# yyamamoto79/guetzli-cuda-opencl

Hardware: AMD Instinct MI355X
Metric: Mpixels/s end-to-end encode @ q=95; achieved HBM GB/s on Butteraugli pass (higher is better)
Workload: dtype f32

## Files before the change

guetzli-cuda-opencl_amd/csrc/kernels/butteraugli_kernels.inc:

```
#pragma once

namespace gz {




constexpr int kIdctM[64] = {
    8192, 11363, 10703, 9633,   8192,  6437,   4433,   2260,   8192, 9633,  4433,  -2259, -8192,
    -11362, -10704, -6436, 8192, 6437, -4433,  -11362, -8192, 2261,   10704,  9633, 8192,  2260,
    -10703, -6436, 8192, 9633,  -4433, -11363, 8192,   -2260, -10703, 6436,   8192, -9633, -4433,
    11363,  8192,  -6437, -4433, 11362, -8192, -2261,  10704, -9633,  8192,   -9633, 4433, 2259,
    -8192,  11362, -10704, 6436, 8192,  -11363, 10703, -9633, 8192,   -6437,  4433,  -2260,
};
typedef short c2l_v2s __attribute__((ext_vector_type(2)));
__device__ __forceinline__ int c2l_dot8(int r, const c2l_v2s (&v)[4], int bias) {
  int acc = bias;
#pragma unroll
  for (int k = 0; k < 4; ++k)
    acc = __builtin_amdgcn_sdot2(c2l_v2s{static_cast<short>(kIdctM[8 * r + 2 * k]),
                                         static_cast<short>(kIdctM[8 * r + 2 * k + 1])},
                                 v[k], acc, false);
  return acc;
}
constexpr int kC2lBlocks = 8;
// ... 166 lines not shown
  scales[static_cast<size_t>(blockIdx.y) * stride + pos] = blur_scale(c_tab.blur[sig], pos, size, &lo, &hi);
}

constexpr int kBlurTile = 256;
constexpr int kBlurLds = 1152;

struct RowsPlain {
  const float* in[kMaxBlurPlanes];
  int w;
  __device__ float at(int p, int y, int x) const { return in[p][static_cast<size_t>(y) * w + x]; }
  __device__ const float* row(int p, int y) const { return in[p] + static_cast<size_t>(y) * w; }
  __device__ static float get(const float* r, int x) { return r[x]; }
  static constexpr bool kPlain = true;
};
struct RowsDiffmap {
  const float* resval;
  int rw;
  __device__ float at(int, int y, int x) const { return resval[static_cast<size_t>(y / 3) * rw + x / 3]; }
  __device__ const float* row(int, int y) const { return resval + static_cast<size_t>(y / 3) * rw; }
  __device__ static float get(const float* r, int x) { return r[x / 3]; }
  static constexpr bool kPlain = false;
};

enum BlurStage : int {
  kBlurRefOpsin = 0, kBlurOpsin, kBlurEdge, kBlurLowFreq, kBlurMask, kBlurDiffmap,
  kBlurLfMask,
};

template <int kSig>
__host__ __device__ constexpr int blur_hstride(int dx) {
  return BlurGeom<kSig>::STEP > 1 ? (dx + 1) & ~1 : dx;
}

template <int kSig> struct HRowRep { static constexpr int N = 1; };
template <> struct HRowRep<kSigDiffmap> { static constexpr int N = 3; };

template <int kSig, int K>
struct H4Geom {
  static constexpr int STEP = BlurGeom<kSig>::STEP, R = BlurGeom<kSig>::R, NT = 2 * R + 1;
  static constexpr int OUT = 64 * K;
  static constexpr int SPAN = OUT * STEP + 2 * R;
  static constexpr int NV = (K + (NT - 1) / STEP + K - 1) / K;
  static constexpr int PMIN = OUT + K * NV;
  static constexpr int PST = STEP == 1 ? (PMIN + 3) / 4 * 4 : ((PMIN + 23) / 32) * 32 + 8;
  static constexpr int LDS = STEP * PST;
};
constexpr int kH4MaxLds = 688;
template <int kSig> struct H4K { static constexpr int K = 2; };

template <int kSig, int K, class Rows>
__device__ __forceinline__ void blur_h4_row(const Rows& rows, float* __restrict__ out, int p, int band,
                                            int y, int w, int lane,
                                            const float* __restrict__ scales, int stride,
                                            float* lds) {
  using G = H4Geom<kSig, K>;
  constexpr int STEP = G::STEP, R = G::R, NT = G::NT, NV = G::NV, PST = G::PST;
  constexpr int IT = (G::SPAN + 63) / 64;
  static_assert(G::LDS <= kH4MaxLds, "H4 LDS region");
  static_assert(K == 2 || K == 4, "2 or 4 outputs per lane");
  const BlurSpec& s = c_tab.blur[kSig];
  const int dx = (w + STEP - 1) / STEP;
  const int ox0 = band * G::OUT;
  const int x_begin = ox0 * STEP - R;
  const float* src = rows.row(p, kSig == kSigDiffmap ? 3 * y : y);
  float v[IT];
  if (Rows::kPlain && x_begin >= 0 && x_begin + IT * 64 <= w) {
    const float* b = src + x_begin + lane;
#pragma unroll
    for (int k = 0; k < IT; ++k) v[k] = b[64 * k];
  } else {
#pragma unroll
    for (int k = 0; k < IT; ++k) {
      const int e = lane + 64 * k, x = x_begin + e;
      const int xc = x < 0 ? 0 : (x < w ? x : w - 1);
      const float t = Rows::get(src, xc);
      v[k] = (e < G::SPAN && x >= 0 && x < w) ? t : 0.0f;
    }
  }
#pragma unroll
  for (int k = 0; k < IT; ++k) {
    const int e = lane + 64 * k;
    if (e < G::SPAN) lds[(e % STEP) * PST + e / STEP] = v[k];
  }
  __builtin_amdgcn_fence(__ATOMIC_RELEASE, "wavefront");
  __builtin_amdgcn_wave_barrier();
  __builtin_amdgcn_fence(__ATOMIC_ACQUIRE, "wavefront");
  float a[STEP][NV * K];
#pragma unroll
  for (int ph = 0; ph < STEP; ++ph)
#pragma unroll
    for (int m = 0; m < NV; ++m) {
      if constexpr (K == 4) {
        const float4 q = *reinterpret_cast<const float4*>(lds + ph * PST + 4 * lane + 4 * m);
        a[ph][4 * m] = q.x;
        a[ph][4 * m + 1] = q.y;
        a[ph][4 * m + 2] = q.z;
        a[ph][4 * m + 3] = q.w;
      } else {
        const float2 q = *reinterpret_cast<const float2*>(lds + ph * PST + 2 * lane + 2 * m);
        a[ph][2 * m] = q.x;
        a[ph][2 * m + 1] = q.y;
      }
    }
  f32x2 s01 = {0.0f, 0.0f}, s23 = {0.0f, 0.0f};
#pragma unroll
  for (int t = 0; t < NT; ++t) {
    const int ph = t % STEP, i = t / STEP;
    const float tap = s.taps[t];
    s01 += f32x2{a[ph][i], a[ph][i + 1]} * tap;
    if constexpr (K == 4) s23 += f32x2{a[ph][i + 2], a[ph][i + 3]} * tap;
  }
  const int ox = ox0 + K * lane;
  const float* sx = scales + static_cast<size_t>(kSig * 2) * stride + ox * STEP;
  float* o = out + static_cast<size_t>(y) * blur_hstride<kSig>(dx) + ox;
  const float r[4] = {s01.x, s01.y, s23.x, s23.y};
#pragma unroll
  for (int j = 0; j < K; ++j)
    if (ox + j < dx) o[j] = r[j] * sx[j * STEP];
}

template <int kStage, class Rows>
__global__ __launch_bounds__(256) void k_blur_h4(Rows rows, BlurPlanes bp, int w, int h,
                                                 const float* __restrict__ scales, int stride) {
  __shared__ __attribute__((aligned(16))) float lds[4][kH4MaxLds];
  const int wv = wave_id(), lane = threadIdx.x & 63;
  const int item = static_cast<int>(blockIdx.x) * 4 + wv;
  if (item >= bp.start[bp.nplanes]) return;
  int q = 0;
  while (q + 1 < bp.nplanes && item >= bp.start[q + 1]) ++q;
  const int local = item - bp.start[q];
  const int band = local % bp.tiles[q], y = local / bp.tiles[q];
#define GZ_H4(S) blur_h4_row<S, H4K<S>::K>(rows, bp.out[q], q, band, y, w, lane, scales, stride, lds[wv])
  if constexpr (kStage == kBlurLowFreq) {
    GZ_H4(kSigLowFreq);
  } else if constexpr (kStage == kBlurMask || kStage == kBlurLfMask) {
    switch (bp.sig[q]) {
      case kSigLowFreq: if constexpr (kStage == kBlurLfMask) GZ_H4(kSigLowFreq); break;
      case kSigMaskX: GZ_H4(kSigMaskX); break;
      case kSigMaskY: GZ_H4(kSigMaskY); break;
      case kSigMaskBSub: GZ_H4(kSigMaskBSub); break;
      default: GZ_H4(kSigMaskB); break;
    }
  } else {
    GZ_H4(kSigDiffmap);
  }
#undef GZ_H4
}

template <int kSig> struct VsRows { static constexpr int N = 8; };
template <> struct VsRows<kSigLowFreq> { static constexpr int N = 16; };
template <int kSig> struct VsAhead { static constexpr int N = 4; };
template <> struct VsAhead<kSigMaskX> { static constexpr int N = 2; };
constexpr int kVsCols = 128;
template <int kSig>
struct VsGeom {
  static constexpr int STEP = BlurGeom<kSig>::STEP, R = BlurGeom<kSig>::R;
  static constexpr int A = 2 * R / STEP + 1;
  static constexpr int S = VsRows<kSig>::N;
  static constexpr int PERIODS = S + A - 1;
};
template <int kSig>
__host__ __device__ constexpr int vstream_segments(int h) {
  return ((h + BlurGeom<kSig>::STEP - 1) / BlurGeom<kSig>::STEP + VsRows<kSig>::N - 1) /
         VsRows<kSig>::N;
}

template <int kSig>
__device__ __forceinline__ void vstream_load(const float* plane, int ds, int h, int y, int ox0,
                                             int ox1, f32x2* v) {
  const int yc = y < 0 ? 0 : (y < h ? y : h - 1);
  const float* r = row_ptr(plane, HRowRep<kSig>::N == 1 ? yc : yc / HRowRep<kSig>::N, ds);
  if constexpr (BlurGeom<kSig>::STEP > 1) {
    *v = *reinterpret_cast<const f32x2*>(r + static_cast<unsigned>(ox0));
  } else {
    *v = f32x2{r[static_cast<unsigned>(ox0)], r[static_cast<unsigned>(ox1)]};
  }
}

template <int kSig, bool kLut = false>
__device__ __forceinline__ void blur_vstream_item(const BlurPlanes& bp, int p, int local, int w,
                                                  int h, int lane, const float* __restrict__ scales,
                                                  int stride) {
  using G = VsGeom<kSig>;
  constexpr int STEP = G::STEP, R = G::R, A = G::A, S = G::S, kVsAhead = VsAhead<kSig>::N;
  const BlurSpec& s = c_tab.blur[kSig];
  const int dx = (w + STEP - 1) / STEP, dy = (h + STEP - 1) / STEP;
  const int segs = vstream_segments<kSig>(h);
  const int seg = local % segs, g = local / segs;
  const int ox = g * kVsCols + 2 * lane;
  const bool in0 = ox < dx, in1 = ox + 1 < dx;
  const int ds = blur_hstride<kSig>(dx);
  const int ox0 = in0 ? ox : (dx - 1) & ~(STEP > 1 ? 1 : 0), ox1 = in1 ? ox + 1 : dx - 1;
  const int oy0 = seg * S;
  const int y_first = oy0 * STEP - R;
  const float* plane = bp.in[p];
  const float* sy = scales + static_cast<size_t>(kSig * 2 + 1) * stride;
  float* out = bp.out[p] + ox;
  float* out2 = kLut && bp.out2[p] ? bp.out2[p] + ox : nullptr;
  const bool lut = kLut && out2 != nullptr;
  f32x2 acc[A];
#pragma unroll
  for (int k = 0; k < A; ++k) acc[k] = f32x2{0.0f, 0.0f};
  f32x2 q[kVsAhead][STEP];
#pragma unroll
  for (int k = 0; k < kVsAhead; ++k)
#pragma unroll
    for (int j = 0; j < STEP; ++j)
      vstream_load<kSig>(plane, ds, h, y_first + k * STEP + j, ox0, ox1, &q[k][j]);
  auto period = [&](int m, f32x2* qm) {
    f32x2 cur[STEP];
#pragma unroll
    for (int j = 0; j < STEP; ++j) {
      const int y = y_first + m * STEP + j;
      const bool yin = y >= 0 && y < h;
      cur[j] = f32x2{masked(qm[j].x, yin), masked(qm[j].y, yin)};
      vstream_load<kSig>(plane, ds, h, y + kVsAhead * STEP, ox0, ox1, &qm[j]);
    }
    acc[0] = f32x2{0.0f, 0.0f};
#pragma unroll
    for (int j = 0; j < STEP; ++j) {
#pragma unroll
      for (int d = 0; d < A; ++d) {
        const int t = d * STEP + j;
        if (t <= 2 * R) acc[d] += cur[j] * s.taps[t];
      }
    }
    const int o = m - (A - 1);
    if (o >= 0 && oy0 + o < dy && o < S) {
      const float sc = sy[(oy0 + o) * STEP];
      const size_t off = static_cast<size_t>(oy0 + o) * dx;
      float* po = out + off;
      const float v0 = acc[A - 1].x * sc, v1 = acc[A - 1].y * sc;
      if (lut) {
        const int c = kSig == kSigMaskX ? 0 : (kSig == kSigMaskY ? 1 : 2);
        float* pd = out2 + off;
        if (in0) mask_lut_pair(c, v0, &po[0], &pd[0]);
        if (in1) mask_lut_pair(c, v1, &po[1], &pd[1]);
      } else {
        if (in0) po[0] = v0;
        if (in1) po[1] = v1;
      }
    }
#pragma unroll
    for (int d = A - 1; d > 0; --d) acc[d] = acc[d - 1];
  };
  for (int m = 0; m < G::PERIODS; m += kVsAhead) {
#pragma unroll
    for (int k = 0; k < kVsAhead; ++k) period(m + k, q[k]);
  }
}

template <int kStage>
__global__ __launch_bounds__(256, 4) void k_blur_vstream(BlurPlanes bp, int w, int h,
                                                      const float* __restrict__ scales, int stride) {
  const int item = static_cast<int>(blockIdx.x) * 4 + wave_id();
  const int lane = threadIdx.x & 63;
  if (item >= bp.start[bp.nplanes]) return;
  int q = 0;
  while (q + 1 < bp.nplanes && item >= bp.start[q + 1]) ++q;
  const int local = item - bp.start[q];
#define GZ_VS(S) blur_vstream_item<S>(bp, q, local, w, h, lane, scales, stride)
#define GZ_VSL(S) blur_vstream_item<S, kStage == kBlurLfMask>(bp, q, local, w, h, lane, scales, stride)
  if constexpr (kStage == kBlurLowFreq) {
    GZ_VS(kSigLowFreq);
  } else if constexpr (kStage == kBlurMask || kStage == kBlurLfMask) {
    switch (bp.sig[q]) {
      case kSigLowFreq: if constexpr (kStage == kBlurLfMask) GZ_VS(kSigLowFreq); break;
      case kSigMaskX: GZ_VSL(kSigMaskX); break;
      case kSigMaskY: GZ_VSL(kSigMaskY); break;
      case kSigMaskBSub: GZ_VSL(kSigMaskBSub); break;
      default: GZ_VSL(kSigMaskB); break;
    }
  } else {
    GZ_VS(kSigDiffmap);
  }
#undef GZ_VS
#undef GZ_VSL
}

constexpr int kB2MaxR = 3;

struct Blur2DPlanes {
  const float* in[6];
  float* out[6];
  int sig[6];
  int nplanes, tiles_x, tiles_y;
};

constexpr int kBsCols = 64 - 2 * kB2MaxR, kBsPf = 8, kBsRows = 32;

template <int kSig>
__device__ __forceinline__ void blur_stream_strip(const float* __restrict__ in, float* __restrict__ out,
                                                  int w, int h, int x0, int y0, int rows, int lane,
                                                  const float* __restrict__ scales, int stride) {
  constexpr int R = BlurGeom<kSig>::R, NT = 2 * R + 1;
  const BlurSpec& s = c_tab.blur[kSig];
  const int x = x0 - kB2MaxR + lane;
  const bool xin = x >= 0 && x < w;
  const int xc = xin ? x : 0;
  const bool emit = lane >= kB2MaxR && lane < kB2MaxR + kBsCols && x < w;
  const float sxv = x < w ? scales[static_cast<size_t>(kSig * 2) * stride + xc] : 0.0f;
  const float* sy = scales + static_cast<size_t>(kSig * 2 + 1) * stride;
  const int y_end = min(y0 + rows, h);
  const int ya = y0 - R, yb = y_end + R;
  auto load = [&](int y) {
    const bool ok = xin && y >= 0 && y < h;
    const int yc = y < 0 ? 0 : (y < h ? y : h - 1);
    const float v = row_ptr(in, yc, w)[static_cast<unsigned>(xc)];
    return masked(v, ok);
  };
  float pm[kBsPf];
#pragma unroll
  for (int k = 0; k < kBsPf; ++k) pm[k] = load(ya + k);
  float hv[NT + 1];
#pragma unroll
  for (int t = 0; t <= NT; ++t) hv[t] = 0.0f;
  for (int y = ya; y < yb; y += 2) {
    const float m0 = pm[0], m1 = pm[1];
#pragma unroll
    for (int k = 0; k + 2 < kBsPf; ++k) pm[k] = pm[k + 2];
    pm[kBsPf - 2] = load(y + kBsPf);
    pm[kBsPf - 1] = load(y + kBsPf + 1);
    float a0[NT], a1[NT];
    a0[R] = m0;
    a1[R] = m1;
#pragma unroll
    for (int k = 1; k <= R; ++k) {
      a0[R + k] = wave_next(a0[R + k - 1]);
      a1[R + k] = wave_next(a1[R + k - 1]);
      a0[R - k] = wave_prev(a0[R - k + 1]);
      a1[R - k] = wave_prev(a1[R - k + 1]);
    }
    f32x2 hs = {0.0f, 0.0f};
#pragma unroll
    for (int t = 0; t < NT; ++t) hs += f32x2{a0[t], a1[t]} * s.taps[t];
    hs *= sxv;
#pragma unroll
    for (int t = 0; t + 2 <= NT; ++t) hv[t] = hv[t + 2];
    hv[NT - 1] = hs.x;
    hv[NT] = hs.y;
    const int yo = y - R;
    if (yo + 1 >= y0) {
      f32x2 acc = {0.0f, 0.0f};
#pragma unroll
      for (int t = 0; t < NT; ++t) acc += f32x2{hv[t], hv[t + 1]} * s.taps[t];
      if (emit && yo >= y0) row_ptr(out, yo, w)[static_cast<unsigned>(x)] = acc.x * sy[yo];
      if (emit && yo + 1 < y_end) row_ptr(out, yo + 1, w)[static_cast<unsigned>(x)] = acc.y * sy[yo + 1];
    }
  }
}

template <int kStage>
__global__ __launch_bounds__(256) void k_blur_stream(Blur2DPlanes bp, int w, int h, int rows,
                                                     const float* __restrict__ scales, int stride) {
  const int lane = threadIdx.x & 63, wv = wave_id();
  const int item = blockIdx.x * 4 + wv;
  const int per_plane = bp.tiles_x * bp.tiles_y;
  if (item >= bp.nplanes * per_plane) return;
  const int p = item / per_plane, t = item % per_plane;
  const int x0 = (t % bp.tiles_x) * kBsCols, y0 = (t / bp.tiles_x) * rows;
#define GZ_BS(S) blur_stream_strip<S>(bp.in[p], bp.out[p], w, h, x0, y0, rows, lane, scales, stride)
  switch (bp.sig[p]) {
    case kSigEdgeX: GZ_BS(kSigEdgeX); break;
    case kSigEdgeY: GZ_BS(kSigEdgeY); break;
    case kSigEdgeB: GZ_BS(kSigEdgeB); break;
    default: GZ_BS(kSigOpsin); break;
  }
#undef GZ_BS
}

constexpr int kOpTX = 64, kOpTY = 32, kOpR = 2;
constexpr int kOpInW = kOpTX + 2 * kOpR, kOpInH = kOpTY + 2 * kOpR;

__global__ __launch_bounds__(256) void k_opsin2d(const float* __restrict__ lin, int w, int h,
                                                 int tiles_x, float* __restrict__ xyb,
                                                 const float* __restrict__ scales, int stride) {
  __shared__ float in_t[kOpInH * kOpInW];
  __shared__ float h_t[3][kOpInH * kOpTX];
  const int x0 = (blockIdx.x % tiles_x) * kOpTX, y0 = (blockIdx.x / tiles_x) * kOpTY;
  const BlurSpec& s = c_tab.blur[kSigOpsin];
  const int ntap = 2 * kOpR + 1;
  const size_t n = static_cast<size_t>(w) * h;
  const float* sx = scales + static_cast<size_t>(kSigOpsin * 2) * stride;
  for (int c = 0; c < 3; ++c) {
    stage_window<kOpInH, kOpInW, kOpInW>(lin + c * n, w, h, x0 - kOpR, y0 - kOpR, in_t);
    __syncthreads();
    #pragma unroll
    for (int k_ = 0; k_ < (kOpInH * kOpTX + 255) / 256; ++k_) {
      const int i = threadIdx.x + 256 * k_;
      if (i >= kOpInH * kOpTX) break;
      const int ry = i / kOpTX, ox = i - ry * kOpTX;
      const int x = x0 + ox;
      float v = 0.0f;
      if (x < w) {
        const float* row = in_t + ry * kOpInW + ox;
        float sum = 0.0f;
        for (int k = 0; k < ntap; ++k) sum += row[k] * s.taps[k];
        v = sum * sx[x];
// ... 1438 lines not shown
```

guetzli-cuda-opencl_amd/csrc/kernels/gz_device.hip:

```cpp
#include <hip/hip_runtime.h>

#include <math.h>
#include <stdio.h>
#include <string.h>
#include <time.h>

#include <algorithm>
#include <chrono>
#include <atomic>
#include <list>
#include <map>
#include <condition_variable>
#include <mutex>
#include <tuple>
#include <string>
#include <vector>

#include "../runtime/engine.h"
#include "../host/frame.h"
#include "../host/thread_pool.h"
#include "gz_math.h"

namespace gz {
__constant__ GzTables c_tab;
// ... 187 lines not shown
    const int dx = (w + st - 1) / st;
    bp.tiles[p] = (dx + kVsCols - 1) / kVsCols;
    bp.start[p + 1] = bp.start[p] + bp.tiles[p] * VStreamSegments(bp.sig[p], h);
  }
  return dim3((bp.start[planes] + 3) / 4);
}
inline int H4Outputs(int sig) {
  switch (sig) {
    case kSigLowFreq: return H4Geom<kSigLowFreq, H4K<kSigLowFreq>::K>::OUT;
    case kSigMaskX: return H4Geom<kSigMaskX, H4K<kSigMaskX>::K>::OUT;
    case kSigMaskY: return H4Geom<kSigMaskY, H4K<kSigMaskY>::K>::OUT;
    case kSigMaskB: return H4Geom<kSigMaskB, H4K<kSigMaskB>::K>::OUT;
    case kSigMaskBSub: return H4Geom<kSigMaskBSub, H4K<kSigMaskBSub>::K>::OUT;
    default: return H4Geom<kSigDiffmap, H4K<kSigDiffmap>::K>::OUT;
  }
}
inline dim3 BlurH4Grid(int w, int h, int planes, BlurPlanes& bp) {
  bp.nplanes = planes;
  bp.start[0] = 0;
  for (int p = 0; p < planes; ++p) {
    const int st = HostTables().blur[bp.sig[p]].step;
    const int dx = (w + st - 1) / st;
    bp.tiles[p] = (dx + H4Outputs(bp.sig[p]) - 1) / H4Outputs(bp.sig[p]);
    const int rep = bp.sig[p] == kSigDiffmap ? HRowRep<kSigDiffmap>::N : 1;
    bp.start[p + 1] = bp.start[p] + bp.tiles[p] * ((h + rep - 1) / rep);
  }
  return dim3((bp.start[planes] + 3) / 4);
}
inline RowsPlain Rows(const BlurPlanes& bp, int w) {
  RowsPlain r{};
  for (int p = 0; p < kMaxBlurPlanes; ++p) r.in[p] = bp.in[p];
  r.w = w;
  return r;
}

}

#define GZ_HIP(call)                                   \
  do {                                                 \
    hipError_t e_ = (call);                            \
    if (e_ != hipSuccess) return Fail(#call, (int)e_); \
  } while (0)
#define GZ_LAUNCH()                                               \
  do {                                                            \
    hipError_t e_ = hipGetLastError();                            \
    if (e_ != hipSuccess) return Fail("kernel launch", (int)e_);  \
  } while (0)

namespace {
std::atomic<int> g_prof_on{0};
std::mutex g_prof_mu;
std::map<std::string, std::pair<long, double>> g_prof;
}

void ProfileEnable(bool on) { g_prof_on.store(on ? 1 : 0); }
void ProfileReset() {
  std::lock_guard<std::mutex> lk(g_prof_mu);
  g_prof.clear();
}
bool ProfileGet(const char* name, long* count, double* total_ms) {
  std::lock_guard<std::mutex> lk(g_prof_mu);
  auto it = g_prof.find(name);
  if (it == g_prof.end()) return false;
  *count = it->second.first;
  *total_ms = it->second.second;
  return true;
}
std::string ProfileNames() {
  std::lock_guard<std::mutex> lk(g_prof_mu);
  std::string out;
  for (auto& kv : g_prof) {
    if (!out.empty()) out += ",";
    out += kv.first;
  }
  return out;
}

void Engine::ProfBegin(const char* name) {
  if (!g_prof_on.load()) return;
  hipEvent_t a = nullptr, b = nullptr;
  if (hipEventCreate(&a) != hipSuccess || hipEventCreate(&b) != hipSuccess) return;
  hipEventRecord(a, static_cast<hipStream_t>(stream_));
  pending_.push_back({name, a, b});
}
void Engine::ProfEnd() {
  if (pending_.empty() || !g_prof_on.load()) return;
  hipEventRecord(static_cast<hipEvent_t>(pending_.back().stop), static_cast<hipStream_t>(stream_));
}
void Engine::ProfMark(const char* name) {
  if (!g_prof_on.load()) return;
  for (auto it = pending_.rbegin(); it != pending_.rend(); ++it)
    if (it->name == name) {
      hipEventRecord(static_cast<hipEvent_t>(it->stop), static_cast<hipStream_t>(stream_));
      return;
    }
}

void Engine::ProfFlush() {
  if (pending_.empty()) return;
  std::lock_guard<std::mutex> lk(g_prof_mu);
  for (auto& p : pending_) {
    float ms = 0.0f;
    if (hipEventSynchronize(static_cast<hipEvent_t>(p.stop)) == hipSuccess &&
        hipEventElapsedTime(&ms, static_cast<hipEvent_t>(p.start), static_cast<hipEvent_t>(p.stop)) == hipSuccess) {
      auto& e = g_prof[p.name];
      e.first += 1;
      e.second += ms;
    }
    hipEventDestroy(static_cast<hipEvent_t>(p.start));
    hipEventDestroy(static_cast<hipEvent_t>(p.stop));
  }
  pending_.clear();
}

#define GZ_TIMED(name, ...) \
  do {                      \
    ProfBegin(name);        \
    __VA_ARGS__;            \
    ProfEnd();              \
    GZ_LAUNCH();            \
  } while (0)

bool Engine::Fail(const char* what, int code) {
  char buf[256];
  snprintf(buf, sizeof(buf), "%s failed: %s (%d)", what,
           hipGetErrorString(static_cast<hipError_t>(code)), code);
  err_ = buf;
  failed_ = true;
  return false;
}

std::unique_ptr<Engine> Engine::Create(int device, int w, int h, std::string* err) {
  std::unique_ptr<Engine> e(new Engine);
  auto fail = [&](const std::string& m) {
    if (err) *err = m;
    return std::unique_ptr<Engine>();
  };
  if (w < 8 || h < 8 || w >= (1 << 16) || h >= (1 << 16)) return fail("unsupported image size");
  int ndev = 0;
  if (hipGetDeviceCount(&ndev) != hipSuccess || ndev == 0) return fail("no HIP device available");
  if (device < 0 || device >= ndev || device >= 64) return fail("bad device index");
  if (hipSetDevice(device) != hipSuccess) return fail("hipSetDevice failed");
  {
    std::lock_guard<std::mutex> lk(g_tab_mu);
    if (!g_tab_uploaded[device]) {
      const GzTables& t = HostTables();
      for (const BlurSpec& b : t.blur)
        if ((kBlurTile - 1) * b.step + 2 * b.radius + 1 + b.step > kBlurLds || 2 * b.radius + 1 > kMaxTaps ||
            b.step < 1 || b.step > 4)
          return fail("blur spec exceeds the tiled kernel's LDS span");
      for (int sig = 0; sig < kNumSigmas; ++sig)
        if (t.blur[sig].step != kBlurGeomStep[sig] || t.blur[sig].radius != kBlurGeomR[sig])
          return fail("blur geometry differs from the compiled BlurGeom table");
      for (int sig = kSigEdgeX; sig <= kSigEdgeB; ++sig)
        if (t.blur[sig].step != 1 || t.blur[sig].radius > kB2MaxR)
          return fail("edge blur spec does not fit the fused 2-D kernel");
      if (hipMemcpyToSymbol(HIP_SYMBOL(c_tab), &t, sizeof(t)) != hipSuccess)
        return fail("table upload failed");
      g_tab_uploaded[device] = true;
    }
  }
  e->device_ = device;
  e->w_ = w;
  e->h_ = h;
  e->bw_ = (w + 7) / 8;
  e->bh_ = (h + 7) / 8;
  e->nb_ = e->bw_ * e->bh_;
  e->rw_ = (w + 2) / 3;
  e->rh_ = (h + 2) / 3;
  e->n_ = static_cast<size_t>(w) * h;
  hipStream_t s;
  if (hipStreamCreateWithFlags(&s, hipStreamNonBlocking) != hipSuccess) return fail("stream");
  e->stream_ = s;
  const size_t n = e->n_, rn = static_cast<size_t>(e->rw_) * e->rh_;
  const size_t nc = static_cast<size_t>(e->nb_) * 64 * 3;
  bool ok = true;
  auto alloc = [&](void** p, size_t bytes) {
    if (ok && hipMalloc(p, bytes) != hipSuccess) ok = false;
    e->bytes_ += bytes;
  };
  alloc(reinterpret_cast<void**>(&e->d_rgb_), 3 * n);
  alloc(reinterpret_cast<void**>(&e->d_orig_), nc * sizeof(int16_t));
  alloc(reinterpret_cast<void**>(&e->d_cur_), nc * sizeof(int16_t));
  alloc(reinterpret_cast<void**>(&e->d_ref_xyb_), 3 * n * 4);
  alloc(reinterpret_cast<void**>(&e->d_lin_), 3 * n * 4);
  alloc(reinterpret_cast<void**>(&e->d_px8_), n * 4);
  alloc(reinterpret_cast<void**>(&e->d_xyb_), 3 * n * 4);
  alloc(reinterpret_cast<void**>(&e->d_m0_), 3 * n * 4);
  alloc(reinterpret_cast<void**>(&e->d_m1_), 3 * n * 4);
  alloc(reinterpret_cast<void**>(&e->d_tmp_), 6 * n * 4);
  alloc(reinterpret_cast<void**>(&e->d_bl_), 6 * n * 4);
  alloc(reinterpret_cast<void**>(&e->d_ma_), 3 * n * 4);
  alloc(reinterpret_cast<void**>(&e->d_mb_), 3 * n * 4);
  alloc(reinterpret_cast<void**>(&e->d_edge_), 3 * rn * 4);
  alloc(reinterpret_cast<void**>(&e->d_dc_), 3 * rn * 4);
  alloc(reinterpret_cast<void**>(&e->d_ac_), 3 * rn * 4);
  alloc(reinterpret_cast<void**>(&e->d_resval_), rn * 4);
  alloc(reinterpret_cast<void**>(&e->d_block_max_), e->nb_ * 4);
  alloc(reinterpret_cast<void**>(&e->d_mask_scale_), 3 * e->nb_ * 4);
  alloc(&e->d_zero_out_, static_cast<size_t>(e->nb_) * 192 * sizeof(CoeffData));
  alloc(reinterpret_cast<void**>(&e->d_zero_count_), static_cast<size_t>(e->nb_) * 4);
  alloc(reinterpret_cast<void**>(&e->d_zero_order_), static_cast<size_t>(e->nb_) * 4);
  alloc(reinterpret_cast<void**>(&e->d_zero_off_), static_cast<size_t>(e->nb_ + 1) * 4);
  alloc(reinterpret_cast<void**>(&e->d_zero_nnz_), static_cast<size_t>(e->nb_) * 4);
  alloc(reinterpret_cast<void**>(&e->d_zero_bins_), 2 * kOrderBins * 4);
  alloc(reinterpret_cast<void**>(&e->d_scan_sums_), (static_cast<size_t>(e->nb_) / 4 + 2) * 4);
  alloc(reinterpret_cast<void**>(&e->d_cand_idx_), static_cast<size_t>(e->nb_) * 192);
  alloc(reinterpret_cast<void**>(&e->d_cand_err_), static_cast<size_t>(e->nb_) * 192 * 4);
  if (ok && hipHostMalloc(reinterpret_cast<void**>(&e->h_zero_off_), static_cast<size_t>(e->nb_ + 1) * 4) != hipSuccess)
    ok = false;
  if (ok && hipHostMalloc(reinterpret_cast<void**>(&e->h_coeffs_), nc * sizeof(int16_t)) != hipSuccess)
    ok = false;
  const size_t stage_groups = (3 * static_cast<size_t>(e->nb_) + kStageBlocks - 1) / kStageBlocks;
  alloc(reinterpret_cast<void**>(&e->d_jhist_), jhist_device_bytes(stage_groups));
  e->jwords_cap_ = static_cast<size_t>(e->nb_) * kCodeWordsPerMcu + 16;
  alloc(reinterpret_cast<void**>(&e->d_jwords_[0]), e->jwords_cap_ * 4);
  alloc(reinterpret_cast<void**>(&e->d_jwords_[1]), e->jwords_cap_ * 4);
  const size_t code_groups = (static_cast<size_t>(e->nb_) + kCodeMcus - 1) / kCodeMcus;
  const size_t jctl_bytes = kCodeFfCopies * 8 + (1 + code_groups / 64 + 2) * 8 + code_groups * 8 +
                            code_groups * 16 + (code_groups + 1) * 4;
  alloc(reinterpret_cast<void**>(&e->d_jctl_), jctl_bytes);
  const size_t jhost_bytes = 4 * (kJCodeHost + kCodeHostFf + (static_cast<size_t>(e->nb_) + kCodeMcus - 1) / kCodeMcus + 16);
  if (ok && hipHostMalloc(reinterpret_cast<void**>(&e->h_jhist_), jhost_bytes, hipHostMallocCoherent) != hipSuccess)
    ok = false;
  if (ok && hipHostGetDevicePointer(reinterpret_cast<void**>(&e->m_jhist_), e->h_jhist_, 0) != hipSuccess)
    ok = false;
  if (ok && (hipMemsetAsync(e->d_jhist_, 0, jhist_device_bytes(stage_groups), s) != hipSuccess ||
             hipMemsetAsync(e->d_jctl_, 0, jctl_bytes, s) != hipSuccess))
    ok = false;
  e->scale_stride_ = (std::max(w, h) + 63) / 64 * 64;
  alloc(reinterpret_cast<void**>(&e->d_scales_), static_cast<size_t>(kNumSigmas) * 2 * e->scale_stride_ * 4);
  const size_t dm_groups = static_cast<size_t>((w + kDmTile - 1) / kDmTile) * ((h + kDmTile - 1) / kDmTile);
  if (ok && hipHostMalloc(reinterpret_cast<void**>(&e->h_block_max_), (e->nb_ + 4 + dm_groups) * 4,
                          hipHostMallocCoherent) != hipSuccess)
    ok = false;
  if (ok && hipHostGetDevicePointer(reinterpret_cast<void**>(&e->m_block_max_), e->h_block_max_, 0) != hipSuccess)
    ok = false;
  const size_t dm_bytes = 4 * kDmMaxWords;
  alloc(reinterpret_cast<void**>(&e->d_dmax_), dm_bytes);
  if (ok && hipMemsetAsync(e->d_dmax_, 0, dm_bytes, s) != hipSuccess) ok = false;

  if (!ok) return fail("device allocation failed");
  e->bytes_ += nc * sizeof(int16_t) + static_cast<size_t>(e->nb_) * 12 + 8192;
  k_blur_scales<<<dim3((e->scale_stride_ + 255) / 256, kNumSigmas * 2), 256, 0, s>>>(
      w, h, e->scale_stride_, e->d_scales_);
  if (hipGetLastError() != hipSuccess || hipStreamSynchronize(s) != hipSuccess)
    return fail("blur scale precompute failed");
  return e;
}

namespace {
std::mutex g_pool_mu;
auto* g_idle = new std::list<std::unique_ptr<Engine>>;
size_t g_idle_bytes = 0;
constexpr size_t kMaxIdlePerKey = 8;

size_t PoolCapBytes() {
  static const size_t cap = [] {
    const char* v = getenv("GZ_ENGINE_POOL_BYTES");
    return v ? static_cast<size_t>(strtoull(v, nullptr, 10)) : (static_cast<size_t>(16) << 30);
  }();
  return cap;
}

void EvictLocked(size_t keep_bytes, std::vector<std::unique_ptr<Engine>>* out) {
  std::map<std::tuple<int, int, int>, size_t> per_key;
  for (auto it = g_idle->begin(); it != g_idle->end();) {
    size_t& n = per_key[std::make_tuple((*it)->device(), (*it)->width(), (*it)->height())];
    if (++n > kMaxIdlePerKey) {
      g_idle_bytes -= (*it)->bytes();
      out->push_back(std::move(*it));
      it = g_idle->erase(it);
    } else {
      ++it;
    }
  }
  while (g_idle_bytes > keep_bytes && !g_idle->empty()) {
    g_idle_bytes -= g_idle->back()->bytes();
    out->push_back(std::move(g_idle->back()));
    g_idle->pop_back();
  }
}
}

std::unique_ptr<Engine> AcquireEngine(int device, int w, int h, std::string* err) {
  {
    std::lock_guard<std::mutex> lk(g_pool_mu);
    for (auto it = g_idle->begin(); it != g_idle->end(); ++it) {
      if ((*it)->device() == device && (*it)->width() == w && (*it)->height() == h) {
        std::unique_ptr<Engine> e = std::move(*it);
        g_idle->erase(it);
        g_idle_bytes -= e->bytes();
        return e;
      }
    }
  }
  return Engine::Create(device, w, h, err);
}

void ReleaseEngine(std::unique_ptr<Engine> e) {
  if (!e || e->failed()) return;
  std::vector<std::unique_ptr<Engine>> evicted;
  {
    std::lock_guard<std::mutex> lk(g_pool_mu);
    g_idle_bytes += e->bytes();
    g_idle->push_front(std::move(e));
// ... 1367 lines not shown
```

guetzli-cuda-opencl_amd/csrc/kernels/gz_math.h:

```cpp
#pragma once

#include <hip/hip_runtime.h>
#include <stdint.h>

namespace gz {

constexpr int kMaxTaps = 72;
constexpr int kNumSigmas = 10;

enum SigmaId : int {
  kSigOpsin = 0,
  kSigEdgeX = 1,
  kSigEdgeY = 2,
  kSigEdgeB = 3,
  kSigLowFreq = 4,
  kSigMaskX = 5,
  kSigMaskY = 6,
  kSigMaskB = 7,
  kSigDiffmap = 8,
  kSigMaskBSub = 9,
};

typedef float f32x2 __attribute__((ext_vector_type(2)));

template <int kSig> struct BlurGeom;
template <> struct BlurGeom<kSigOpsin> { static constexpr int R = 2, STEP = 1; };
template <> struct BlurGeom<kSigEdgeX> { static constexpr int R = 3, STEP = 1; };
template <> struct BlurGeom<kSigEdgeY> { static constexpr int R = 1, STEP = 1; };
template <> struct BlurGeom<kSigEdgeB> { static constexpr int R = 1, STEP = 1; };
template <> struct BlurGeom<kSigLowFreq> { static constexpr int R = 31, STEP = 4; };
template <> struct BlurGeom<kSigMaskX> { static constexpr int R = 21, STEP = 3; };
template <> struct BlurGeom<kSigMaskY> { static constexpr int R = 32, STEP = 4; };
template <> struct BlurGeom<kSigMaskB> { static constexpr int R = 10, STEP = 1; };
template <> struct BlurGeom<kSigDiffmap> { static constexpr int R = 19, STEP = 2; };
template <> struct BlurGeom<kSigMaskBSub> { static constexpr int R = 10, STEP = 3; };
constexpr int kBlurGeomR[kNumSigmas] = {2, 3, 1, 1, 31, 21, 32, 10, 19, 10};
constexpr int kBlurGeomStep[kNumSigmas] = {1, 1, 1, 1, 4, 3, 4, 1, 2, 3};

#define GZ_BLUR_SWITCH(sig, F)            \
  switch (sig) {                          \
    case kSigOpsin: F(kSigOpsin); break;  \
    case kSigEdgeX: F(kSigEdgeX); break;  \
    case kSigEdgeY: F(kSigEdgeY); break;  \
    case kSigEdgeB: F(kSigEdgeB); break;  \
    case kSigLowFreq: F(kSigLowFreq); break; \
    case kSigMaskX: F(kSigMaskX); break;  \
    case kSigMaskY: F(kSigMaskY); break;  \
    case kSigMaskB: F(kSigMaskB); break;  \
    case kSigMaskBSub: F(kSigMaskBSub); break; \
    default: F(kSigDiffmap); break;       \
  }

struct BlurSpec {
  int radius;
  int step;
  float border_ratio;
  float weight_no_border;
  float taps[kMaxTaps];
};

struct GzTables {
  float srgb[256];
  int cr_r[256], cb_b[256], cr_g[256], cb_g[256];
  float hf_dx[21], hf_dy[21], lf_dy[21];
  double hf_dy_d[21], lf_dy_d[21];
  float mask_lut[6][512];
  float block_csf[37];
  double block_csf_d[37];
  double ac_w_d[3][33];
  float csf_xb[2][37];
  float zeroing_csf[192];
  uint8_t zigzag[64];
  uint8_t old_csf[64];
  int idct[64];
  float opsin8_scale[8];
  BlurSpec blur[kNumSigmas];
};

constexpr int kMaxBlurPlanes = 9;
struct BlurPlanes {
  const float* in[kMaxBlurPlanes];
  float* out[kMaxBlurPlanes];
  float* out2[kMaxBlurPlanes];
  int sig[kMaxBlurPlanes];
  int nplanes;
  int tiles[kMaxBlurPlanes];
  int start[kMaxBlurPlanes + 1];
};

extern __constant__ GzTables c_tab;

struct BlockId {
  int x, y, z;
};
__device__ __forceinline__ BlockId xcd_block_id() {
  const unsigned gx = gridDim.x, gy = gridDim.y;
  const unsigned n = gx * gy * gridDim.z;
  const unsigned lin = (blockIdx.z * gy + blockIdx.y) * gx + blockIdx.x;
  const unsigned q = n / 8, r = n % 8, xcd = lin % 8, k = lin / 8;
  const unsigned id = (xcd < r ? xcd * (q + 1) : r * (q + 1) + (xcd - r) * q) + k;
  return BlockId{static_cast<int>(id % gx), static_cast<int>((id / gx) % gy),
                 static_cast<int>(id / (gx * gy))};
}


__device__ __forceinline__ int wave_id() { return __builtin_amdgcn_readfirstlane(threadIdx.x >> 6); }

template <class T>
__device__ __forceinline__ T* row_ptr(T* base, int y, int w) {
  return base + static_cast<size_t>(y) * w;
}

__device__ __forceinline__ float masked(float v, bool keep) {
  return __int_as_float(__float_as_int(v) & (keep ? -1 : 0));
}

__device__ __forceinline__ float wave_next(float v) {
  return __int_as_float(__builtin_amdgcn_update_dpp(__float_as_int(v), __float_as_int(v), 0x130, 0xf, 0xf, true));
}
__device__ __forceinline__ float wave_prev(float v) {
  return __int_as_float(__builtin_amdgcn_update_dpp(__float_as_int(v), __float_as_int(v), 0x138, 0xf, 0xf, true));
}


__device__ __forceinline__ float interp_f(const float* a, int size, float sx) {
  const float ix = fabsf(sx);
  const int base = static_cast<int>(ix);
  float res;
  if (base >= size - 1) {
    res = a[size - 1];
  } else {
    const float mix = ix - base;
    res = a[base] + mix * (a[base + 1] - a[base]);
  }
  return sx < 0 ? -res : res;
}

__device__ __forceinline__ float interp_pair_f(const float2* t, int size, float sx) {
  const float ix = fabsf(sx);
  const int base = static_cast<int>(ix);
  const float mix = __builtin_amdgcn_fractf(ix);
  const float2 p = t[base < size - 1 ? base : size - 1];
  const float res = p.x + mix * p.y;
  return sx < 0 ? -res : res;
}

__device__ __forceinline__ float sqrt_cr_big(float x) {
  const float s = __builtin_amdgcn_sqrtf(x);
  const float dn = __uint_as_float(__float_as_uint(s) - 1u);
  const float up = __uint_as_float(__float_as_uint(s) + 1u);
  const float r = fmaf(-dn, s, x) <= 0.0f ? dn : s;
  return fmaf(-up, s, x) > 0.0f ? up : r;
}
__device__ __forceinline__ bool sqrt_needs_scale(float x) {
  return __float_as_uint(x) - 1u < 0x0f7fffffu;
}

__device__ __forceinline__ float interp_clamp_neg_f(const float* a, int size, float sx) {
  if (sx < 0) sx = 0;
  const float ix = fabsf(sx);
  const int base = static_cast<int>(ix);
  if (base >= size - 1) return a[size - 1];
  const float mix = ix - base;
  return a[base] + mix * (a[base + 1] - a[base]);
}

__device__ __forceinline__ double interp_d(const double* a, int size, double sx) {
  const double ix = fabs(sx);
  const int base = static_cast<int>(ix);
  double res;
  if (base >= size - 1) {
    res = a[size - 1];
  } else {
    const double mix = ix - base;
    res = a[base] + mix * (a[base + 1] - a[base]);
  }
  return sx < 0 ? -res : res;
}

__device__ __forceinline__ void lowfreq_sq_zero_f(float x, float y, float z, float factor,
                                                  float res[3], const float* lf_dy = c_tab.lf_dy) {
  z += 0.0812519812628f * y;
  const float vz = z * 7.34905756986f;
  const float vx = x * 6.64482198135f;
  const float vy = interp_f(lf_dy, 21, y * 0.837846224276f);
  res[0] += factor * vx * vx;
  res[1] += factor * vy * vy;
  res[2] += factor * vz * vz;
}

__device__ __forceinline__ float interp_tab(const float* a, int size, float sx) { return interp_f(a, size, sx); }
__device__ __forceinline__ float interp_tab(const float2* t, int size, float sx) {
  return interp_pair_f(t, size, sx);
}

template <class Tab = float>
__device__ __forceinline__ void lowfreq_vals_f(float x, float y, float z, float v[3],
                                               const Tab* lf_dy = c_tab.lf_dy) {
  z += 0.0812519812628f * y;
  v[2] = z * 7.34905756986f;
  v[0] = x * 6.64482198135f;
  v[1] = interp_tab(lf_dy, 21, y * 0.837846224276f);
}

template <class Tab = float>
__device__ __forceinline__ void lowfreq_sq_f(const float a[3], const float b[3], float factor,
                                             float res[3], const Tab* lf_dy = c_tab.lf_dy) {
  float v0[3];
  lowfreq_vals_f(a[0], a[1], a[2], v0, lf_dy);
  if (b[0] == 0.0f && b[1] == 0.0f && b[2] == 0.0f) {
    res[0] += factor * v0[0] * v0[0];
    res[1] += factor * v0[1] * v0[1];
// ... 344 lines not shown
```

Measured before the change: 302.2.

## Use symmetric tap pairs with packed-multiply inline asm in vertical blur stream

Loads only half of the symmetric blur taps into SGPR pairs and multiplies with v_pk_mul_f32 using op_sel to pick the high or low tap, instead of scalar multiplies against the full tap table. Adds sched_barrier fences per group of four products and fully unrolls the period loop for step-1 sigmas. The goal is fewer scalar loads and VALU ops, and better scheduling, in the vertical streaming blur. A host check rejects tables whose taps are not bitwise symmetric, and the taps array is aligned to 8 bytes. The inline asm constrains register allocation and the full unroll may raise code size and register pressure.

```diff
diff --git a/guetzli-cuda-opencl_amd/csrc/kernels/butteraugli_kernels.inc b/guetzli-cuda-opencl_amd/csrc/kernels/butteraugli_kernels.inc
--- a/guetzli-cuda-opencl_amd/csrc/kernels/butteraugli_kernels.inc
+++ b/guetzli-cuda-opencl_amd/csrc/kernels/butteraugli_kernels.inc
@@ -342,6 +342,8 @@
 template <int kSig> struct VsAhead { static constexpr int N = 4; };
 template <> struct VsAhead<kSigMaskX> { static constexpr int N = 2; };
 constexpr int kVsCols = 128;
+constexpr int kVsGroup = 4;
+constexpr int kVsFenceMask = 0x4 | 0x10;
 template <int kSig>
 struct VsGeom {
   static constexpr int STEP = BlurGeom<kSig>::STEP, R = BlurGeom<kSig>::R;
@@ -365,6 +367,17 @@
   } else {
     *v = f32x2{r[static_cast<unsigned>(ox0)], r[static_cast<unsigned>(ox1)]};
   }
+}
+
+template <int kHigh>
+__device__ __forceinline__ f32x2 pk_mul_tap(f32x2 pair, f32x2 v) {
+  f32x2 r;
+  if constexpr (kHigh) {
+    asm volatile("v_pk_mul_f32 %0, %1, %2 op_sel:[1,0] op_sel_hi:[1,1]" : "=v"(r) : "s"(pair), "v"(v));
+  } else {
+    asm volatile("v_pk_mul_f32 %0, %1, %2 op_sel_hi:[0,1]" : "=v"(r) : "s"(pair), "v"(v));
+  }
+  return r;
 }
 
 template <int kSig, bool kLut = false>
@@ -391,6 +404,11 @@
   f32x2 acc[A];
 #pragma unroll
   for (int k = 0; k < A; ++k) acc[k] = f32x2{0.0f, 0.0f};
+  constexpr int kPairs = R / 2 + 1;
+  static_assert(2 * kPairs <= kMaxTaps, "tap pairs inside the table");
+  f32x2 tp[kPairs];
+#pragma unroll
+  for (int i = 0; i < kPairs; ++i) tp[i] = *reinterpret_cast<const f32x2*>(&s.taps[2 * i]);
   f32x2 q[kVsAhead][STEP];
 #pragma unroll
   for (int k = 0; k < kVsAhead; ++k)
@@ -410,11 +428,22 @@
 #pragma unroll
     for (int j = 0; j < STEP; ++j) {
 #pragma unroll
-      for (int d = 0; d < A; ++d) {
-        const int t = d * STEP + j;
-        if (t <= 2 * R) acc[d] += cur[j] * s.taps[t];
-      }
-    }
+      for (int d0 = 0; d0 < A; d0 += kVsGroup) {
+        f32x2 prod[kVsGroup];
+#pragma unroll
+        for (int k = 0; k < kVsGroup; ++k) {
+          const int t = (d0 + k) * STEP + j, th = t <= R ? t : 2 * R - t;
+          if (d0 + k < A && t <= 2 * R)
+            prod[k] = (th & 1) ? pk_mul_tap<1>(tp[th / 2], cur[j]) : pk_mul_tap<0>(tp[th / 2], cur[j]);
+        }
+#pragma unroll
+        for (int k = 0; k < kVsGroup; ++k)
+          if (d0 + k < A && (d0 + k) * STEP + j <= 2 * R) acc[d0 + k] += prod[k];
+        __builtin_amdgcn_sched_barrier(kVsFenceMask);
+      }
+    }
+#pragma unroll
+    for (int d = 0; d < A; ++d) asm volatile("" : "+v"(acc[d]));
     const int o = m - (A - 1);
     if (o >= 0 && oy0 + o < dy && o < S) {
       const float sc = sy[(oy0 + o) * STEP];
@@ -434,6 +463,7 @@
 #pragma unroll
     for (int d = A - 1; d > 0; --d) acc[d] = acc[d - 1];
   };
+#pragma unroll(STEP == 1 ? G::PERIODS : 1)
   for (int m = 0; m < G::PERIODS; m += kVsAhead) {
 #pragma unroll
     for (int k = 0; k < kVsAhead; ++k) period(m + k, q[k]);
diff --git a/guetzli-cuda-opencl_amd/csrc/kernels/gz_device.hip b/guetzli-cuda-opencl_amd/csrc/kernels/gz_device.hip
--- a/guetzli-cuda-opencl_amd/csrc/kernels/gz_device.hip
+++ b/guetzli-cuda-opencl_amd/csrc/kernels/gz_device.hip
@@ -363,6 +363,10 @@
       for (int sig = 0; sig < kNumSigmas; ++sig)
         if (t.blur[sig].step != kBlurGeomStep[sig] || t.blur[sig].radius != kBlurGeomR[sig])
           return fail("blur geometry differs from the compiled BlurGeom table");
+      for (const BlurSpec& b : t.blur)
+        for (int i = 0; i < b.radius; ++i)
+          if (memcmp(&b.taps[i], &b.taps[2 * b.radius - i], sizeof(float)) != 0)
+            return fail("blur taps are not bitwise symmetric");
       for (int sig = kSigEdgeX; sig <= kSigEdgeB; ++sig)
         if (t.blur[sig].step != 1 || t.blur[sig].radius > kB2MaxR)
           return fail("edge blur spec does not fit the fused 2-D kernel");
diff --git a/guetzli-cuda-opencl_amd/csrc/kernels/gz_math.h b/guetzli-cuda-opencl_amd/csrc/kernels/gz_math.h
--- a/guetzli-cuda-opencl_amd/csrc/kernels/gz_math.h
+++ b/guetzli-cuda-opencl_amd/csrc/kernels/gz_math.h
@@ -56,8 +56,9 @@
   int step;
   float border_ratio;
   float weight_no_border;
-  float taps[kMaxTaps];
+  alignas(8) float taps[kMaxTaps];
 };
+static_assert(sizeof(BlurSpec) == 16 + 4 * kMaxTaps, "BlurSpec layout");
 
 struct GzTables {
   float srgb[256];
```

Result: slower. 198.7 (-34.2%).
